# seongsujeong/MIMC3

Hardware: AMD Instinct MI355X
Metric: grid-points/s (DLC NCC match) (higher is better)
Workload: dtype u8

## Files before the change

### mimc3_amd/csrc/match_px_kernel.hip

```cpp
#include <hip/hip_runtime.h>
#include <type_traits>
#include <atomic>
#include <mutex>
#include <stdint.h>
#include <stdlib.h>
#include <stdio.h>
#include "match_kernel.h"
#include "sat_kernel.h"

#ifndef MIMC3_XY_ACC
#define MIMC3_XY_ACC 2
#endif
#ifndef MIMC3_SAT_DEFER
#define MIMC3_SAT_DEFER -1
#endif
#ifndef MIMC3_WN
#define MIMC3_WN 1
#endif
#ifndef MIMC3_NULL_FLAGS
#define MIMC3_NULL_FLAGS 1
#endif
#ifndef MIMC3_OPQ_SMALL
#define MIMC3_OPQ_SMALL 1
#endif
#ifndef MIMC3_FAST_REPLAY
#define MIMC3_FAST_REPLAY 1
#endif
#ifndef MIMC3_WIDE_REPLAY
#define MIMC3_WIDE_REPLAY 1
#endif
#ifndef MIMC3_GC
#define MIMC3_GC 1
#endif
#ifndef MIMC3_STAGE_KB
#define MIMC3_STAGE_KB 8
#endif
#ifndef MIMC3_EVEN_PITCH
#define MIMC3_EVEN_PITCH 0
#endif
#ifndef MIMC3_FAST_BATCH
#define MIMC3_FAST_BATCH 64
#endif

namespace mimc3 {

static constexpr float kUnknown = 3.0f;
static constexpr float kWanted = 4.0f;

__device__ __forceinline__ uint32_t dot4(uint32_t a, uint32_t b, uint32_t c) { return __builtin_amdgcn_udot4(a, b, c, false); }
__device__ __forceinline__ uint32_t alignb(uint32_t hi, uint32_t lo, uint32_t s) { return __builtin_amdgcn_alignbyte(hi, lo, s); }
__device__ __forceinline__ uint32_t nz80(uint32_t v) { return (((v & 0x7f7f7f7fu) + 0x7f7f7f7fu) | v) & 0x80808080u; }
typedef unsigned short nzff_us2_t __attribute__((ext_vector_type(2)));
__device__ __forceinline__ uint32_t nzff(uint32_t v)
{
    const uint32_t e = (v & 0x00ff00ffu) + 0x7fff7fffu;
    const nzff_us2_t k = {0x7f00, 0x7f00};
    const uint32_t o = __builtin_bit_cast(uint32_t, __builtin_elementwise_add_sat(__builtin_bit_cast(nzff_us2_t, v), k));
    return __builtin_amdgcn_perm(o, e, 0x0b090a08u);
}

template <int LPC>
__device__ __forceinline__ uint32_t group_sum(uint32_t v)
{
    int x = (int)v;
    x += __builtin_amdgcn_update_dpp(0, x, 0xB1, 0xF, 0xF, true);
    x += __builtin_amdgcn_update_dpp(0, x, 0x4E, 0xF, 0xF, true);
    if (LPC >= 8) x += __builtin_amdgcn_update_dpp(0, x, 0x141, 0xF, 0xF, true);
    if (LPC >= 16) x += __builtin_amdgcn_update_dpp(0, x, 0x140, 0xF, 0xF, true);
    if (LPC >= 32) x += __shfl_xor(x, 16, 64);
    if (LPC >= 64) x += __shfl_xor(x, 32, 64);
    return (uint32_t)x;
}
__device__ __forceinline__ int wave_sum_i(int v)
{
#pragma unroll
    for (int o = 32; o > 0; o >>= 1) v += __shfl_xor(v, o, 64);
    return v;
}

__device__ __forceinline__ void argmax_row16(float &v, int &i)
{
#define MIMC3_ARGMAX_STEP(ctrl)                                                                           \
    {                                                                                                     \
        const float ov = __int_as_float(__builtin_amdgcn_update_dpp(0, __float_as_int(v), ctrl, 0xF, 0xF, true)); \
        const int oi = __builtin_amdgcn_update_dpp(0, i, ctrl, 0xF, 0xF, true);                           \
        const bool t = (ov > v) || (ov == v && oi < i);                                                   \
        v = t ? ov : v; i = t ? oi : i;                                                                   \
    }
    MIMC3_ARGMAX_STEP(0xB1) MIMC3_ARGMAX_STEP(0x4E) MIMC3_ARGMAX_STEP(0x141) MIMC3_ARGMAX_STEP(0x140)
#undef MIMC3_ARGMAX_STEP
}

enum { M_FAST = 0, M_CHIPNULL = 1, M_GENERAL = 2, M_XY = 3, M_WN = 4, M_GC = 5 };

template <class S> struct AccT { uint32_t n; S sx, sy, sxx, syy, sxy; };

__device__ __forceinline__ double dpp_add_f64(double x, int ctrl_sel)
{
    const long long b = __double_as_longlong(x);
    int lo = (int)(b & 0xffffffffll), hi = (int)(b >> 32);
    int olo, ohi;
    switch (ctrl_sel) {
    case 0: olo = __builtin_amdgcn_update_dpp(0, lo, 0xB1, 0xF, 0xF, true); ohi = __builtin_amdgcn_update_dpp(0, hi, 0xB1, 0xF, 0xF, true); break;
    case 1: olo = __builtin_amdgcn_update_dpp(0, lo, 0x4E, 0xF, 0xF, true); ohi = __builtin_amdgcn_update_dpp(0, hi, 0x4E, 0xF, 0xF, true); break;
    case 2: olo = __builtin_amdgcn_update_dpp(0, lo, 0x141, 0xF, 0xF, true); ohi = __builtin_amdgcn_update_dpp(0, hi, 0x141, 0xF, 0xF, true); break;
    default: olo = __builtin_amdgcn_update_dpp(0, lo, 0x140, 0xF, 0xF, true); ohi = __builtin_amdgcn_update_dpp(0, hi, 0x140, 0xF, 0xF, true); break;
    }
    return x + __longlong_as_double(((long long)ohi << 32) | (unsigned int)olo);
}

struct PxU8 {
    static constexpr int BPP = 1, G = 4, LOG2G = 2;
    static constexpr bool SRC16 = false;
    static constexpr bool INTEGER = true;
    static constexpr bool SAT = true;
    static constexpr bool SATZ = false;
    static constexpr bool SAT_CHIP = true;
    static constexpr bool WN = true;
    typedef unsigned long long SatT;
    __device__ static __forceinline__ unsigned long long sat_s(SatT q) { return (uint32_t)q & ((1u << kSatSqShift8) - 1u); }
    __device__ static __forceinline__ unsigned long long sat_ss(SatT q) { return (uint32_t)(q >> kSatSqShift8) & ((1u << (kSatNullShift8 - kSatSqShift8)) - 1u); }
    __device__ static __forceinline__ int sat_nulls(SatT q) { return (int)(q >> kSatNullShift8); }
    __device__ static __forceinline__ void sat_win_sums(uint32_t &sy, uint32_t &syy, SatT q, int, int, int, double) { sy = (uint32_t)sat_s(q); syy = (uint32_t)sat_ss(q); }
    __device__ static __forceinline__ uint32_t px_at(const unsigned char *p) { return *p; }
    typedef uint32_t Sum;
    static constexpr uint32_t lowmask_c(int npx) { return npx >= 4 ? 0xffffffffu : ((1u << (8 * npx)) - 1u); }
    __device__ static __forceinline__ uint32_t lowmask(int npx) { return npx >= 4 ? 0xffffffffu : ((1u << (8 * npx)) - 1u); }
    __device__ static __forceinline__ int npx(uint32_t m) { return __popc(m & 0x01010101u); }
    __device__ static __forceinline__ int nbad(uint32_t v, uint32_t keep, float) { return npx(keep) - __popc(nz80(v) >> 7); }
    __device__ static __forceinline__ int nexcl(uint32_t v, uint32_t keep, float thr) { return nbad(v, keep, thr); }
    __device__ static __forceinline__ uint32_t sanitize(uint32_t a, float) { return a; }
    __device__ static __forceinline__ bool maybe_excl(uint32_t v, uint32_t keep, float) { return ((v - 0x01010101u) & ~v & 0x80808080u & keep) != 0u; }
    __device__ static __forceinline__ void chip_acc(Sum &sx, Sum &sxx, uint32_t a) { sx = dot4(a, 0x01010101u, sx); sxx = dot4(a, a, sxx); }
    template <int MODE, bool OPQ>
    __device__ static __forceinline__ void task(AccT<Sum> &acc, uint32_t a, uint32_t pad01, uint32_t padff, bool static_pad, uint32_t bw, float)
    {
        if (MODE == M_XY) {
            if (static_pad) acc.sxy = dot4(a, bw, acc.sxy); else acc.sy = dot4(a, bw, acc.sy);
            return;
        }
        if (MODE == M_WN) {
            const uint32_t am = a & nzff(bw);
            acc.sx = dot4(am, 0x01010101u, acc.sx);
            acc.sxx = dot4(am, a, acc.sxx);
            acc.sxy = dot4(a, bw, acc.sxy);
            return;
        }
        if (MODE == M_GC && static_pad) {
            const uint32_t mbff = nzff(bw);
            const uint32_t am = a & mbff;
            acc.n += (uint32_t)__popc(padff == 0xffffffffu ? mbff : (mbff & padff));
            acc.sx = dot4(am, 0x01010101u, acc.sx);
            acc.sy = dot4(pad01, bw, acc.sy);
            acc.sxy = dot4(a, bw, acc.sxy);
            acc.sxx = dot4(am, a, acc.sxx);
            acc.syy = dot4(padff == 0xffffffffu ? bw : (bw & padff), bw, acc.syy);
            return;
        }
        if (OPQ && !(MODE == M_FAST && static_pad)) asm volatile("" : "+v"(a));
        const uint32_t mf = (MODE == M_FAST && static_pad) ? padff : nzff(a);
        if (MODE == M_FAST) {
            const uint32_t m01 = static_pad ? pad01 : (mf & 0x01010101u);
            const uint32_t mff = static_pad ? padff : mf;
            acc.sy = dot4(m01, bw, acc.sy);
            acc.syy = dot4((static_pad && padff == 0xffffffffu) ? bw : (bw & mff), bw, acc.syy);
            acc.sxy = dot4(a, bw, acc.sxy);
        } else if (MODE == M_CHIPNULL) {
            const uint32_t bm = bw & mf;
            acc.sy = dot4(bm, 0x01010101u, acc.sy);
            acc.syy = dot4(bm, bw, acc.syy);
            acc.sxy = dot4(a, bw, acc.sxy);
        } else {
            const uint32_t mbff = nzff(bw);
            const uint32_t am = a & mbff, bm = bw & mf;
            acc.n += (uint32_t)__popc(mbff & mf);
            acc.sx = dot4(am, 0x01010101u, acc.sx);
            acc.sy = dot4(bm, 0x01010101u, acc.sy);
            acc.sxy = dot4(a, bw, acc.sxy);
            acc.sxx = dot4(am, a, acc.sxx);
            acc.syy = dot4(bm, bw, acc.syy);
        }
    }
    __device__ static __forceinline__ uint32_t n_units(uint32_t n) { return n >> 3; }
    template <int LPC> __device__ static __forceinline__ Sum gsum(Sum v) { return group_sum<LPC>(v); }
    typedef uint32_t Store;
    __device__ static __forceinline__ Store bits(Sum v) { return v; }
    __device__ static __forceinline__ float ncc(const Store *sp, double, double, int, int)
    {
        const double dn = (double)sp[0], dsx = (double)sp[1], dsy = (double)sp[2];
        const double num = dn * (double)sp[5] - dsx * dsy;
        const double den = sqrt((dn * (double)sp[3] - dsx * dsx) * (dn * (double)sp[4] - dsy * dsy));
        return (float)(num / den);
    }
};

typedef unsigned short us2_t __attribute__((ext_vector_type(2)));
__device__ __forceinline__ uint32_t dot2(uint32_t a, uint32_t b, uint32_t c)
{
    return __builtin_amdgcn_udot2(__builtin_bit_cast(us2_t, a), __builtin_bit_cast(us2_t, b), c, false);
}
__device__ __forceinline__ uint32_t nz8000(uint32_t v) { return (((v & 0x7fff7fffu) + 0x7fff7fffu) | v) & 0x80008000u; }
__device__ __forceinline__ uint32_t ffff_from8000(uint32_t t) { return t | (t - (t >> 15)); }
__device__ __forceinline__ unsigned long long dpp_add_u64(unsigned long long x, int ctrl_sel)
{
    int lo = (int)(uint32_t)x, hi = (int)(uint32_t)(x >> 32);
    int olo, ohi;
    switch (ctrl_sel) {
    case 0: olo = __builtin_amdgcn_update_dpp(0, lo, 0xB1, 0xF, 0xF, true); ohi = __builtin_amdgcn_update_dpp(0, hi, 0xB1, 0xF, 0xF, true); break;
    case 1: olo = __builtin_amdgcn_update_dpp(0, lo, 0x4E, 0xF, 0xF, true); ohi = __builtin_amdgcn_update_dpp(0, hi, 0x4E, 0xF, 0xF, true); break;
    case 2: olo = __builtin_amdgcn_update_dpp(0, lo, 0x141, 0xF, 0xF, true); ohi = __builtin_amdgcn_update_dpp(0, hi, 0x141, 0xF, 0xF, true); break;
    default: olo = __builtin_amdgcn_update_dpp(0, lo, 0x140, 0xF, 0xF, true); ohi = __builtin_amdgcn_update_dpp(0, hi, 0x140, 0xF, 0xF, true); break;
    }
    return x + (((unsigned long long)(uint32_t)ohi << 32) | (uint32_t)olo);
}
struct PxU16 {
    static constexpr int BPP = 2, G = 2, LOG2G = 1;
    static constexpr bool SRC16 = false;
    static constexpr bool INTEGER = true;
    static constexpr bool SAT = true;
    static constexpr bool SATZ = true;
    static constexpr bool SAT_CHIP = true;
    static constexpr bool WN = true;
    typedef unsigned long long SatT;
    __device__ static __forceinline__ unsigned long long sat_s(SatT q) { return q & ((1ull << kSatSqShift16) - 1ull); }
    __device__ static __forceinline__ unsigned long long sat_ss(SatT q) { return q >> kSatSqShift16; }
    __device__ static __forceinline__ int sat_nulls(SatT) { return 0; }
    __device__ static __forceinline__ void sat_win_sums(unsigned long long &sy, unsigned long long &syy, SatT q, int, int, int, double) { sy = sat_s(q); syy = sat_ss(q); }
    __device__ static __forceinline__ uint32_t px_at(const unsigned char *p) { return *reinterpret_cast<const unsigned short *>(p); }
    typedef unsigned long long Sum;
    static constexpr uint32_t lowmask_c(int npx) { return npx >= 2 ? 0xffffffffu : (npx == 1 ? 0x0000ffffu : 0u); }
    __device__ static __forceinline__ uint32_t lowmask(int npx) { return npx >= 2 ? 0xffffffffu : (npx == 1 ? 0x0000ffffu : 0u); }
    __device__ static __forceinline__ int npx(uint32_t m) { return __popc(m & 0x00010001u); }
    __device__ static __forceinline__ int nbad(uint32_t v, uint32_t keep, float) { return npx(keep) - __popc(nz8000(v) >> 15); }
    __device__ static __forceinline__ int nexcl(uint32_t v, uint32_t keep, float thr) { return nbad(v, keep, thr); }
    __device__ static __forceinline__ uint32_t sanitize(uint32_t a, float) { return a; }
// ... 186 lines not shown
        const double sxx = __longlong_as_double((long long)sp[3]), syy = __longlong_as_double((long long)sp[4]);
        const double sxy = __longlong_as_double((long long)sp[5]);
        const double num = dn * sxy - sx * sy;
        const double den = sqrt((dn * sxx - sx * sx) * (dn * syy - sy * sy));
        return (float)(num / den);
    }
};

struct PxF32i : PxF32 {
    static constexpr bool SAT = true, SATZ = false, SAT_CHIP = true;
    static constexpr bool WN = true;
    typedef Sat2 SatT;
    __device__ static __forceinline__ double sat_s(const SatT &q) { return (double)(q.a & ((1ull << kSatNullShiftF) - 1ull)); }
    __device__ static __forceinline__ double sat_ss(const SatT &q) { return (double)q.b; }
    __device__ static __forceinline__ int sat_nulls(const SatT &q) { return (int)(q.a >> kSatNullShiftF); }
    __device__ static __forceinline__ void sat_win_sums(double &sy, double &syy, const SatT &q, int, int, int, double sc) { sy = sat_s(q) * sc; syy = sat_ss(q) * (sc * sc); }
    template <int MODE, bool OPQ>
    __device__ static __forceinline__ void task(AccT<Sum> &acc, uint32_t au, uint32_t p01, uint32_t pff, bool static_pad, uint32_t bu, float thr)
    {
        if (MODE == M_XY) {
            const double pr = (double)(__uint_as_float(au) * __uint_as_float(bu));
            if (static_pad) acc.sxy += pr; else acc.sy += pr;
            return;
        }
        if (MODE == M_WN) {
            const float a = __uint_as_float(au), b = __uint_as_float(bu);
            const float a2 = (b != 0.0f) ? a : 0.0f;
            acc.sx += (double)a2; acc.sxx += (double)(a2 * a2); acc.sxy += (double)(a * b);
            return;
        }
        PxF32::template task<MODE, OPQ>(acc, au, p01, pff, static_pad, bu, thr);
    }
};

template <class P_, int OCW_, int LPC_, int NW_ = 1, int MINW_ = 2, bool CHL_ = false, bool MANY_ = false, bool COMPACT_ = false>
struct PxCfg {
    typedef P_ P;
    static constexpr bool COMPACT = COMPACT_;
    static constexpr bool SAT_DEFER = std::is_same<P_, PxU8>::value && NW_ == 1;
    static constexpr int MINW = MINW_;
    static constexpr int OCW = OCW_, LPC = LPC_;
    static constexpr int NW = NW_, NT = 64 * NW_;
    static constexpr int CW = 2 * OCW + 1, NPX = CW * CW;
    static constexpr int GPR = (CW + P::G - 1) / P::G;
    static constexpr bool SHORT = CW < LPC;
    static constexpr int RF = SHORT ? 1 : CW / LPC;
    static constexpr int REM = SHORT ? 0 : CW - RF * LPC;
    static constexpr int TT = (REM * GPR + LPC - 1) / LPC;
    static constexpr int LASTN = CW - P::G * (GPR - 1);
    static constexpr uint32_t LASTFF = P::lowmask_c(LASTN);
    static constexpr uint32_t LAST01 = LASTFF & 0x01010101u;
    static constexpr int CPR = 64 / LPC;
    static constexpr bool WN = P_::WN && (!std::is_same<P_, PxU8>::value || ((SHORT ? 1 : CW / LPC_) >= 2 && !((LPC_ >= 64) && P_::INTEGER)));
    static constexpr bool kOpqSmall = MIMC3_OPQ_SMALL && ((std::is_same<P_, PxU8>::value && OCW_ == 16) || (std::is_same<P_, PxU8o>::value && (OCW_ == 15 || OCW_ == 16)));
    static constexpr bool OPQ = LPC_ >= 64 || kOpqSmall;
    static constexpr bool SPARSE = (LPC_ >= 64) && P::INTEGER;
    static constexpr int CPITCH = 4 * GPR;
    static constexpr bool CHIP_LDS = CHL_;
    static constexpr bool CHIP_COPY = SPARSE || CHIP_LDS;
    static constexpr bool MANYP = MANY_;
    static constexpr bool REC = false;
    static constexpr bool SHORTCUT = !MANY_ && ((OCW_ == 16 && !std::is_same<P_, PxF32>::value) ||
                                                (OCW_ == 7 && (std::is_same<P_, PxU8>::value || std::is_same<P_, PxU8o>::value || std::is_same<P_, PxF32>::value)));
    static constexpr bool one_pad_task_per_lane()
    {
        for (int ln = 0; ln < LPC_; ln++) {
            int cnt = 0;
            for (int k = 0; k < TT; k++) {
                const int tt = ln + LPC_ * k;
                if (tt < REM * GPR && tt % GPR == GPR - 1) cnt++;
            }
            if (cnt > 1) return false;
        }
        return true;
    }
    static constexpr bool FULLTAIL = SPARSE && !CHIP_LDS && TT >= 4 && LASTN < P::G && one_pad_task_per_lane();
};
template <class C0>
struct PxRec : C0 {
    static constexpr bool REC = true;
};
static constexpr int kLwCap = 1024;
static constexpr int kLcCap = 512;

struct U8Point {
    int dx2, dy2, Dx2, Dy2, csx, csy, ncell;
    int sh;
    int PW;
    int zrow;
    float thr;
};

template <class C, int MODE, bool REDUCE = true, bool FULLTAIL = false>
__device__ __forceinline__ AccT<typename C::P::Sum> eval_round(const unsigned char *W, const U8Point &pt, int cx, int cy, int l,
                                          const uint32_t (&A)[C::RF > 0 ? C::RF : 1][C::GPR],
                                          const uint32_t (&AT)[C::TT > 0 ? C::TT : 1],
                                          const int (&toff)[C::TT > 0 ? C::TT : 1],
                                          AccT<typename C::P::Sum> acc = AccT<typename C::P::Sum>{0, 0, 0, 0, 0, 0},
                                          const unsigned char *CH = nullptr)
{
    typedef typename C::P P;
    [[maybe_unused]] const typename P::Sum sy_in = acc.sy;
    const int X = pt.sh + cx;
    const uint32_t s = (uint32_t)((X & (P::G - 1)) * P::BPP);
    const unsigned char *base = W + cy * pt.PW + 4 * (X >> P::LOG2G);
    constexpr int NLD = C::GPR + (P::G > 1 ? 1 : 0);
    if constexpr (C::CHIP_LDS) {
        constexpr int KC = 8;
#pragma unroll
        for (int i = 0; i < C::RF; i++) {
            const bool idle = C::SHORT && l >= C::CW;
            const uint32_t *rp = reinterpret_cast<const uint32_t *>(idle ? W + pt.zrow * pt.PW : base + (l + C::LPC * i) * pt.PW);
            const uint32_t *cp = reinterpret_cast<const uint32_t *>(CH + (idle ? 0 : (l + C::LPC * i)) * C::CPITCH);
#pragma unroll 1
            for (int j0 = 0; j0 < C::GPR - 1; j0 += KC) {
                uint32_t w[KC + 1], a[KC];
#pragma unroll
                for (int k = 0; k <= KC; k++) w[k] = rp[j0 + k];
#pragma unroll
                for (int k = 0; k < KC; k++) a[k] = (j0 + k < C::GPR - 1 && !idle) ? cp[j0 + k] : 0u;
#pragma unroll
                for (int k = 0; k < KC; k++) {
                    const uint32_t bw = (P::G > 1) ? alignb(w[k + 1], w[k], s) : w[k];
                    if (j0 + k < C::GPR - 1) P::template task<MODE, C::OPQ>(acc, a[k], 0x01010101u, 0xffffffffu, true, bw, pt.thr);
                }
            }
            {
                constexpr int j = C::GPR - 1;
                const uint32_t w0 = rp[j], w1 = (P::G > 1) ? rp[j + 1] : 0u;
                const uint32_t bw = (P::G > 1) ? alignb(w1, w0, s) : w0;
                const uint32_t av = idle ? 0u : cp[j];
                P::template task<MODE, C::OPQ>(acc, av, C::LAST01, C::LASTFF, true, bw, pt.thr);
            }
        }
    } else {
#pragma unroll
    for (int i = 0; i < C::RF; i++) {
        const uint32_t *rp = reinterpret_cast<const uint32_t *>(base + (l + C::LPC * i) * pt.PW);
        if (C::SHORT && l >= C::CW) rp = reinterpret_cast<const uint32_t *>(W + pt.zrow * pt.PW);
        uint32_t w[NLD];
#pragma unroll
        for (int j = 0; j < NLD; j++) w[j] = rp[j];
#pragma unroll
        for (int j = 0; j < C::GPR; j++) {
            const uint32_t bw = (P::G > 1) ? alignb(w[j + (P::G > 1 ? 1 : 0)], w[j], s) : w[j];
            const uint32_t p01 = (j == C::GPR - 1) ? C::LAST01 : 0x01010101u;
            const uint32_t pff = (j == C::GPR - 1) ? C::LASTFF : 0xffffffffu;
            if constexpr (MODE == M_XY) P::template task<M_XY, C::OPQ>(acc, A[i][j], 0, 0, (MIMC3_XY_ACC < 2) || ((i * C::GPR + j) & 1) == 0, bw, pt.thr);
            else P::template task<MODE, C::OPQ>(acc, A[i][j], p01, pff, true, bw, pt.thr);
        }
    }
    }
#pragma unroll
    for (int k = 0; k < C::TT; k++) {
        const uint32_t *rp = reinterpret_cast<const uint32_t *>(base + toff[k]);
        const uint32_t bw = (P::G > 1) ? alignb(rp[P::G > 1 ? 1 : 0], rp[0], s) : rp[0];
        uint32_t av = AT[k];
        if constexpr (C::CHIP_LDS) {
            const int tt = l + C::LPC * k;
            av = tt < C::REM * C::GPR ? *reinterpret_cast<const volatile uint32_t *>(CH + (C::RF * C::LPC + tt / C::GPR) * C::CPITCH + 4 * (tt % C::GPR)) : 0u;
        }
        if constexpr (MODE == M_XY) {
            P::template task<M_XY, C::OPQ>(acc, av, 0, 0, (MIMC3_XY_ACC < 2) || (k & 1) == 0, bw, pt.thr);
        }
        else if constexpr (FULLTAIL && MODE == M_FAST) {
            uint32_t bwt = bw;
            if (k == C::TT - 1 && (C::REM * C::GPR) % C::LPC != 0) bwt = (l + C::LPC * k < C::REM * C::GPR) ? bw : 0u;
            P::template task<M_FAST, C::OPQ>(acc, av, P::BPP == 1 ? 0x01010101u : 0x00010001u, 0xffffffffu, true, bwt, pt.thr);
        }
        else P::template task<MODE, C::OPQ>(acc, av, 0, 0, false, bw, pt.thr);
    }
    if constexpr (MODE == M_XY && MIMC3_XY_ACC >= 2) { acc.sxy += acc.sy - sy_in; acc.sy = sy_in; }
    if (MODE == M_GENERAL || MODE == M_GC) acc.n = P::n_units(acc.n);
    if (!REDUCE) return acc;
    acc.sxy = P::template gsum<C::LPC>(acc.sxy);
    if (MODE != M_XY && MODE != M_WN) { acc.sy = P::template gsum<C::LPC>(acc.sy); acc.syy = P::template gsum<C::LPC>(acc.syy); }
    if (MODE == M_WN) { acc.sx = P::template gsum<C::LPC>(acc.sx); acc.sxx = P::template gsum<C::LPC>(acc.sxx); }
    if (MODE == M_GENERAL || MODE == M_GC) {
        acc.n = group_sum<C::LPC>(acc.n); acc.sx = P::template gsum<C::LPC>(acc.sx); acc.sxx = P::template gsum<C::LPC>(acc.sxx);
    }
    return acc;
}

static constexpr int kStatW = 20;
#ifndef MIMC3_SUM_BATCH
#define MIMC3_SUM_BATCH 32
#endif
static constexpr int kSumBatch = MIMC3_SUM_BATCH;

#define MIMC3_STAMP(i)                                                                         \
    if (p.stats) {                                                                             \
        const unsigned long long t_now = __builtin_amdgcn_s_memtime();                         \
        if (threadIdx.x == 0) p.stats[kStatW * (size_t)blockIdx.x + i] += t_now - t_prev;                   \
        t_prev = t_now;                                                                        \
    }

template <class C>
__global__ __launch_bounds__(C::NT, C::MINW) void match_ncc_dlc_px(MatchU8Args p)
{
    typedef typename C::P P;
    typedef typename P::Sum Sum;
    constexpr bool kSat = P::SAT && !C::MANYP, kSatChip = P::SAT_CHIP && kSat, kSatZ = P::SATZ && kSat;
    unsigned long long t_prev = p.stats ? __builtin_amdgcn_s_memtime() : 0ull;
    extern __shared__ __attribute__((aligned(16))) unsigned char smem[];
    const int tid = threadIdx.x, lane = tid & 63, wave = tid >> 6;
    const int l = lane & (C::LPC - 1), grp = lane / C::LPC;
    constexpr int OCW = C::OCW, CW = C::CW, GPR = C::GPR, NT = C::NT, NW = C::NW;

    int gidx = blockIdx.x;
    constexpr bool kRec = C::REC;
    static_assert(!kRec || (std::is_same<P, PxU8>::value && !C::MANYP), "point records: the 8-bit policy's plain forms");
    [[maybe_unused]] uint32_t recw = 0u;
    auto rec = [&](int k) __attribute__((always_inline)) -> uint32_t { return (uint32_t)__builtin_amdgcn_readlane((int)recw, k); };
    if (kRec || p.point_list) {
        const int cnt = *p.point_count;
        if (gidx >= cnt) return;
        const int per = cnt >> 3;
        if (gidx < per * 8) gidx = (gidx & 7) * per + (gidx >> 3);
        if constexpr (kRec) {
            static_assert(sizeof(U8PointRec) == 64 && offsetof(U8PointRec, chipQ) == 40, "the dword numbers below");
            recw = reinterpret_cast<const uint32_t *>(p.point_recs + gidx)[lane & 15];
            if (rec(8) & kRecDone) return;
            gidx = (int)rec(0);
        } else gidx = p.point_list[gidx];
    } else {
        const int nb = gridDim.x, per = nb >> 3;
        if (per > 0 && gidx < per * 8) gidx = (gidx & 7) * per + (gidx >> 3);
    }
    if (gidx >= p.N) return;
    if (p.point_flags && p.point_flags[gidx] != (uint8_t)p.flag_value) return;
// ... 416 lines not shown
                    exc_chip += nzc;
                    if constexpr (C::SPARSE) {
                        if (wave == 0 && rowok && nzc) {
                            int at = atomicAdd(&qcnt[17], nzc);
                            if (at + nzc > kLcCap) qcnt[18] = 1;
                            else {
#pragma unroll
                                for (int k = 0; k < P::G; k++) {
                                    const uint32_t pm = P::lowmask(1) << (8 * P::BPP * k);
                                    if ((pff & pm) && !(a & pm)) nl_put(Lc, at++, (uint32_t)(P::G * j + k), (uint32_t)(l + C::LPC * i));
                                }
                            }
                        }
                    }
                }
            }
#pragma unroll
            for (int k = 0; k < C::TT; k++) {
                const int tt = l + C::LPC * k;
                const bool on = tt < C::REM * GPR;
                const int j = on ? tt % GPR : 0;
                const uint32_t pff = on ? ((j == GPR - 1) ? C::LASTFF : 0xffffffffu) : 0u;
                if (P::maybe_excl(AT[k], pff, pt.thr)) {
                    bad_chip += P::nbad(AT[k], pff, pt.thr);
                    const int nzc = P::nexcl(AT[k], pff, pt.thr);
                    exc_chip += nzc;
                    if constexpr (C::FULLTAIL || (kSat && C::SPARSE)) {
                        if (wave == 0 && on && nzc) {
                            int at = atomicAdd(&qcnt[17], nzc);
                            if (at + nzc > kLcCap) qcnt[18] = 1;
                            else {
#pragma unroll
                                for (int q = 0; q < P::G; q++) {
                                    const uint32_t pm = P::lowmask(1) << (8 * P::BPP * q);
                                    if ((pff & pm) && !(AT[k] & pm)) nl_put(Lc, at++, (uint32_t)(P::G * j + q), (uint32_t)(C::RF * C::LPC + tt / GPR));
                                }
                            }
                        }
                    }
                }
            }
        }
        if constexpr (kSatChip) {
            bad_chip = exc_chip = chip_nulls;
            SX = (Sum)P::sat_s(chipQ); SXX = (Sum)P::sat_ss(chipQ);
            if constexpr (!P::INTEGER) { SX = (Sum)((double)SX * sc_chip); SXX = (Sum)((double)SXX * (sc_chip * sc_chip)); }
        } else {
            bad_chip = (int)group_sum<C::LPC>((uint32_t)bad_chip); exc_chip = (int)group_sum<C::LPC>((uint32_t)exc_chip);
            SX = P::template gsum<C::LPC>(SX); SXX = P::template gsum<C::LPC>(SXX);
        }
    }
    const uint32_t NV = (uint32_t)(C::NPX - exc_chip);
    const int clean_mode = (exc_chip == 0) ? M_FAST : M_CHIPNULL;
    MIMC3_STAMP(1)
    if (p.debug_stop == 2) { if (tid == 0) p.out[3 * (size_t)gidx] = (float)((uint32_t)P::bits(SX) + (uint32_t)P::bits(SXX) + bad_chip + A[0][0] + AT[0]); return; }
    __syncthreads();
    const bool sparse_on = C::SPARSE && qcnt[18] == 0;
    const int nLw = sparse_on ? qcnt[16] : 0, nLc = sparse_on ? qcnt[17] : 0;
    (void)nLw; (void)nLc;
    if (p.stats && tid == 0) {
        p.stats[kStatW * (size_t)blockIdx.x + 11] += sparse_on ? 1 : 0;
        p.stats[kStatW * (size_t)blockIdx.x + 12] += (unsigned)nLw; p.stats[kStatW * (size_t)blockIdx.x + 13] += (unsigned)nLc;
    }

    {
        const float max_ratio = 0.8f;
        const float rc = (float)bad_chip / (float)(CW * CW);
        const float rw = (float)bad_win / (float)(pt.Dx2 * pt.Dy2);
        if (rc > max_ratio || rw > max_ratio) {
            if (tid == 0) {
                const float nanv = __builtin_nanf("");
                p.out[3 * (size_t)gidx + 0] = nanv;
                p.out[3 * (size_t)gidx + 1] = nanv;
                p.out[3 * (size_t)gidx + 2] = -3.0f;
            }
            return;
        }
    }
    static_assert(OCW >= 2, "T4 cmap cells are reachable by the fit only when ocw == 1; not instantiated");
    auto box_clean = [&](int cx, int cy) __attribute__((always_inline)) -> bool {
        if (!full_win && (cx == pt.csx - 2 || cy == pt.csy - 2)) return false;
        if (win_clean) return true;
        return (cx > nbx1) || (cx + CW - 1 < nbx0) || (cy > nby1) || (cy + CW - 1 < nby0);
    };

    auto request = [&](int cx, int cy) __attribute__((always_inline)) {
        if (!claim(cx, cy)) return;
        if constexpr (C::COMPACT) {
            const int slot = atomicAdd(&qcnt[2], 1);
            if (slot >= p.lds_nslot) { qcnt[3] = 1; return; }
            give_slot(cx, cy, slot);
        }
        const bool cl = box_clean(cx, cy);
        const uint32_t q = (uint32_t)atomicAdd(&qcnt[0], cl ? 1 : (1 << 16));
        const int ia = (int)(q & 0xffffu), ib = (int)(q >> 16);
        if (ia + ib + 1 > lcap) { qcnt[3] = 1; return; }
        const uint16_t packed = (uint16_t)((cy << 8) | cx);
        if (cl) list[ia] = packed; else list[lcap - 1 - ib] = packed;
    };
    auto inside = [&](int pu, int pvv) __attribute__((always_inline)) -> bool {
        return !(pu - OCW <= 1 || pu + OCW >= pt.Dx2 - 1 || pvv - OCW <= 1 || pvv + OCW >= pt.Dy2 - 1);
    };
    auto scan9 = [&](int cu, int cv, float &sm) __attribute__((always_inline)) -> int {
        float v[9];
#pragma unroll
        for (int j = 0; j < 9; j++) v[j] = lookup(cu + (j / 3 - 1) - OCW, cv + (j % 3 - 1) - OCW);
// ... 20 lines not shown
        if constexpr (C::COMPACT) {
            slot0 = atomicAdd(&qcnt[2], __popc(won));
            if (slot0 + __popc(won) > p.lds_nslot) { qcnt[3] = 1; return; }
        }
        const uint32_t row_t4 = (!full_win && cy0 == pt.csy - 3) ? 4u : 0u;
        const bool col_t4 = !full_win && cx0 == pt.csx - 3;
        uint32_t cl;
        if (win_clean) {
            cl = (7u & ~row_t4) * (col_t4 ? 0x09u : 0x49u);
        } else {
            uint32_t row_ok = 0u;
#pragma unroll
            for (int k = 0; k < 3; k++) {
                const int cy = cy0 + k - 1;
                row_ok |= (cy > nby1 || cy + CW - 1 < nby0) ? (1u << k) : 0u;
            }
            cl = 0u;
#pragma unroll
            for (int i = 0; i < 3; i++) {
                const int cx = cx0 + i - 1;
                const bool col_ok = cx > nbx1 || cx + CW - 1 < nbx0;
                const uint32_t part = (i == 2 && col_t4) ? 0u : ((col_ok ? 7u : row_ok) & ~row_t4);
                cl |= part << (3 * i);
            }
        }
        const uint32_t wa = won & cl, wb = won & ~cl;
        const int na = __popc(wa), nb = __popc(wb);
        const uint32_t q = (uint32_t)atomicAdd(&qcnt[0], na | (nb << 16));
        int ia = (int)(q & 0xffffu), ib = (int)(q >> 16);
        if (ia + ib + na + nb > lcap) { qcnt[3] = 1; return; }
#pragma unroll
        for (int j = 0; j < 9; j++) {
            if (!((won >> j) & 1u)) continue;
            const int cx = cx0 + (j / 3 - 1), cy = cy0 + (j % 3 - 1);
            const uint16_t packed = (uint16_t)((cy << 8) | cx);
            if ((wa >> j) & 1u) list[ia++] = packed; else list[lcap - 1 - ib++] = packed;
            if constexpr (C::COMPACT) give_slot(cx, cy, slot0++);
        }
    };
    for (int k = tid; k < npiv; k += NT) {
        const int pu = pivs[2 * k] + pt.dx2, pvv = pivs[2 * k + 1] + pt.dy2;
        if (!inside(pu, pvv)) continue;
        request9(pu - OCW, pvv - OCW);
    }
    __syncthreads();
    if (p.debug_stop == 3) return;
    MIMC3_STAMP(2)

    constexpr bool kAPark = (C::LPC >= 32) && P::INTEGER;
    constexpr bool kSatDefer = MIMC3_SAT_DEFER < 0 ? C::SAT_DEFER : (MIMC3_SAT_DEFER != 0);
    auto evaluate = [&](const uint16_t *ids, int dir, int cnt, int mode) __attribute__((always_inline)) {
        const bool dirty_list = (mode == M_GENERAL);
        const bool wn_ok = kSat && C::WN && MIMC3_WN && dirty_list && exc_chip == 0;
        uint32_t ew[4] = {0xffffffffu, 0xffffffffu, 0xffffffffu, 0xffffffffu}, ec[2] = {0xffffffffu, 0xffffffffu};
        if constexpr (C::SPARSE) {
            if (sparse_on && cnt > 0) {
                if (dirty_list) {
#pragma unroll
                    for (int k = 0; k < 4; k++) if (l + k * C::LPC < nLw) ew[k] = nl_get(Lw, l + k * C::LPC);
                }
#pragma unroll
                for (int k = 0; k < 2; k++) if (l + k * C::LPC < nLc) ec[k] = nl_get(Lc, l + k * C::LPC);
            }
        }
        constexpr int kFastBatch = (6 * kSumBatch < MIMC3_FAST_BATCH) ? 6 * kSumBatch : MIMC3_FAST_BATCH;
        const bool one_word = kSat && !kAPark && NT == 64 && mode == M_FAST && kFastBatch > kSumBatch;
        const int batch_cells = one_word ? kFastBatch : kSumBatch;
        for (int b0 = 0; b0 < cnt; b0 += batch_cells) {
            const int nb = (cnt - b0) < batch_cells ? (cnt - b0) : batch_cells;
            [[maybe_unused]] SatT cellQ{}, q00{}, q01{}, q10{}, q11{};
            [[maybe_unused]] int cellZ = 0;
            if constexpr (kSat) {
                const bool need = mode == M_FAST || (C::SPARSE && sparse_on) || (dirty_list && wn_ok);
                if (need && tid < nb) {
                    const uint32_t pk = ids[dir * (b0 + tid)];
                    const SatT *r0 = sat_win + (size_t)(wv0 + (int)((pk >> 8) & 0xffu)) * p.sat_ws + (wu0 + (int)(pk & 0xffu)), *r1 = r0 + (size_t)CW * p.sat_ws;
                    q00 = r0[0]; q01 = r0[CW]; q10 = r1[0]; q11 = r1[CW];
                    if (!kSatDefer) cellQ = q11 - q01 - q10 + q00;
                    if constexpr (kSatZ) {
                        if (dirty_list) cellZ = (int)sat_box(satz_win, p.sat_ws, wu0 + (int)(pk & 0xffu), wv0 + (int)((pk >> 8) & 0xffu), CW, CW);
                    }
                }
            }
            [[maybe_unused]] unsigned char *nzf = reinterpret_cast<unsigned char *>(&qcnt[24]);
            constexpr bool kNullFlags = C::SPARSE && kSat && !kSatDefer && kSumBatch <= 32 && MIMC3_NULL_FLAGS;
            const bool flags_on = kNullFlags && 3 * CW * CW <= pt.Dx2 * pt.Dy2;
            if constexpr (kNullFlags) {
                if (dirty_list && sparse_on && flags_on) {
                    if (tid < nb) nzf[tid] = (unsigned char)((kSatZ ? cellZ : P::sat_nulls(cellQ)) != 0);
                    __syncthreads();
                }
            }
            for (int r0 = 0; r0 < nb; r0 += C::CPR * NW) {
                const int slot = r0 + wave * C::CPR + grp;
                const bool on = slot < nb;
                const uint32_t pk = on ? ids[dir * (b0 + slot)] : 0x00000101u;
                const int cx = (int)(pk & 0xffu), cy = (int)((pk >> 8) & 0xffu);
                AccT<Sum> acc;
                bool six = dirty_list;
                bool done = false;
                bool wn_round = false;
                if constexpr (C::SPARSE) {
                    if (sparse_on && !(dirty_list && !full_win && (cx == pt.csx - 2 || cy == pt.csy - 2))) {
                        AccT<Sum> a0{0, 0, 0, 0, 0, 0};
                        uint32_t cn = 0;
                        Sum csx = 0, csxx = 0, csy = 0, csyy = 0;
                        auto corr_w = [&](const uint32_t (&e)[4]) __attribute__((always_inline)) {
                            uint32_t av[4];
                            bool in[4];
#pragma unroll
                            for (int k = 0; k < 4; k++) {
                                const int ddx = (int)(e[k] & 0xffffu) - cx, ddy = (int)(e[k] >> 16) - cy;
                                in[k] = (unsigned)ddx < (unsigned)CW && (unsigned)ddy < (unsigned)CW;
                                av[k] = P::px_at(CH + (in[k] ? (int)__umul24(ddy, C::CPITCH) + ddx * P::BPP : 0));
                            }
#pragma unroll
                            for (int k = 0; k < 4; k++) {
                                const uint32_t a1 = in[k] ? av[k] : 0u;
                                cn += a1 ? 1u : 0u; csx += a1; csxx += (Sum)__umul24(a1, a1);
                            }
                        };
                        const unsigned char *Wc = W + cy * pt.PW + (pt.sh + cx) * P::BPP;
                        auto corr_c = [&](const uint32_t (&e)[2]) __attribute__((always_inline)) {
                            uint32_t bv[2];
#pragma unroll
                            for (int k = 0; k < 2; k++) {
                                const bool ok = e[k] != 0xffffffffu;
                                bv[k] = P::px_at(Wc + (ok ? (int)__umul24(e[k] >> 16, pt.PW) + (int)(e[k] & 0xffffu) * P::BPP : 0));
                                bv[k] = ok ? bv[k] : 0u;
                            }
#pragma unroll
                            for (int k = 0; k < 2; k++) { csy += bv[k]; csyy += (Sum)__umul24(bv[k], bv[k]); }
                        };
                        bool wnull = dirty_list;
                        if constexpr (kNullFlags) { if (flags_on) wnull = dirty_list && on && nzf[slot] != 0; }
                        six = wnull;
                        if (wnull) {
                            corr_w(ew);
                            for (int i0 = l + 4 * C::LPC; i0 < nLw; i0 += 4 * C::LPC) {
                                uint32_t e[4];
#pragma unroll
                                for (int k = 0; k < 4; k++) e[k] = (i0 + k * C::LPC < nLw) ? nl_get(Lw, i0 + k * C::LPC) : 0xffffffffu;
                                corr_w(e);
                            }
                        }
                        if (nLc > 0) {
                            corr_c(ec);
                            for (int i0 = l + 2 * C::LPC; i0 < nLc; i0 += 2 * C::LPC) {
                                uint32_t e[2];
#pragma unroll
                                for (int k = 0; k < 2; k++) e[k] = (i0 + k * C::LPC < nLc) ? nl_get(Lc, i0 + k * C::LPC) : 0xffffffffu;
                                corr_c(e);
                            }
                        }
                        if constexpr (C::FULLTAIL && !kSat) {
                            const int X = pt.sh + cx;
                            const uint32_t sft = (uint32_t)((X & (P::G - 1)) * P::BPP);
                            const uint32_t *rp = reinterpret_cast<const uint32_t *>(W + cy * pt.PW + 4 * (X >> P::LOG2G) + (padoff >= 0 ? padoff : 0));
                            const uint32_t pb = padoff >= 0 ? (alignb(rp[1], rp[0], sft) & ~C::LASTFF) : 0u;
                            P::chip_acc(csy, csyy, pb);
                        }
                        constexpr bool kFold = sizeof(Sum) == 4;
                        if (kFold) { a0.sy = (Sum)0 - csy; a0.syy = (Sum)0 - csyy; }
                        acc = eval_round<C, kSat ? M_XY : M_FAST, false, C::FULLTAIL>(W, pt, cx, cy, l, A, AT, toff, a0, CH);
                        if (!kFold) { acc.sy -= csy; acc.syy -= csyy; }
                        acc.n = 0u - cn; acc.sx = (Sum)0 - csx; acc.sxx = (Sum)0 - csxx;
                        done = true;
                    } else {
                        six = dirty_list;
                    }
                }
                if (!done) {
                    if (mode == M_FAST) acc = eval_round<C, kSat ? M_XY : M_FAST, !kAPark>(W, pt, cx, cy, l, A, AT, toff, AccT<Sum>{0, 0, 0, 0, 0, 0}, CH);
                    else if (mode == M_CHIPNULL) acc = eval_round<C, M_CHIPNULL, !kAPark>(W, pt, cx, cy, l, A, AT, toff, AccT<Sum>{0, 0, 0, 0, 0, 0}, CH);
                    else {
                        if constexpr (kSat) {
                            const bool t4 = on && !full_win && (cx == pt.csx - 2 || cy == pt.csy - 2);
                            wn_round = wn_ok && __ballot(t4) == 0ull;
                        }
                        if (kSat && wn_round) acc = eval_round<C, kSat ? M_WN : M_GENERAL, !kAPark>(W, pt, cx, cy, l, A, AT, toff, AccT<Sum>{0, 0, 0, 0, 0, 0}, CH);
                        else if (MIMC3_GC && exc_chip == 0) acc = eval_round<C, M_GC, !kAPark>(W, pt, cx, cy, l, A, AT, toff, AccT<Sum>{0, 0, 0, 0, 0, 0}, CH);
                        else acc = eval_round<C, M_GENERAL, !kAPark>(W, pt, cx, cy, l, A, AT, toff, AccT<Sum>{0, 0, 0, 0, 0, 0}, CH);
                    }
                }
                Store *sp = sums + 6 * slot;
                if constexpr (kAPark) {
                    const bool lead = on && (l & 15) == 0;
                    const Sum rsxy = P::template gsum<16>(acc.sxy);
                    if (lead) atomicAdd(&sp[5], P::bits(rsxy));
                    if (!kSat || (done ? nLc > 0 : (mode != M_FAST && !wn_round))) {
                        const Sum rsy = P::template gsum<16>(acc.sy), rsyy = P::template gsum<16>(acc.syy);
                        if (lead) { atomicAdd(&sp[2], P::bits(rsy)); atomicAdd(&sp[4], P::bits(rsyy)); }
                    }
                    if (six) {
                        const Sum rsx = P::template gsum<16>(acc.sx), rsxx = P::template gsum<16>(acc.sxx);
                        if (lead) { atomicAdd(&sp[1], P::bits(rsx)); atomicAdd(&sp[3], P::bits(rsxx)); }
                        if (!wn_round) {
                            const uint32_t rn = group_sum<16>(acc.n);
                            if (lead) atomicAdd(&sp[0], (Store)rn);
                        }
                    }
                } else {
                    if (kSat && mode == M_FAST) {
                        if (on && l == 0) { if (one_word) sums[slot] = P::bits(acc.sxy); else sp[5] = P::bits(acc.sxy); }
                    } else {
                        if (mode != M_GENERAL) { acc.n = NV; acc.sx = SX; acc.sxx = SXX; }
                        if (on && l == 0) {
                            if (kSat && wn_round) { sp[1] = P::bits(acc.sx); sp[3] = P::bits(acc.sxx); sp[5] = P::bits(acc.sxy); }
                            else { sp[0] = (Store)acc.n; sp[1] = P::bits(acc.sx); sp[2] = P::bits(acc.sy); sp[3] = P::bits(acc.sxx); sp[4] = P::bits(acc.syy); sp[5] = P::bits(acc.sxy); }
                        }
                    }
                }
            }
            __syncthreads();
            if (tid < nb) {
                if (kSatDefer) cellQ = q11 - q01 - q10 + q00;
                const uint32_t pk = ids[dir * (b0 + tid)];
                const int cx = (int)(pk & 0xffu), cy = (int)((pk >> 8) & 0xffu);
                Store *sp = sums + 6 * tid;
                Store v[6] = {0, 0, 0, 0, 0, 0};
                if (one_word) v[5] = sums[tid];
                else { v[0] = sp[0]; v[1] = sp[1]; v[2] = sp[2]; v[3] = sp[3]; v[4] = sp[4]; v[5] = sp[5]; }
                bool wn_cell = false;
                if constexpr (kSat) {
                    if (wn_ok) {
                        const bool t4 = !full_win && (cx == pt.csx - 2 || cy == pt.csy - 2);
                        const unsigned long long tm = __ballot(t4);
                        wn_cell = ((tm >> (tid & ~(C::CPR - 1))) & ((1ull << C::CPR) - 1ull)) == 0ull;
                        if (C::SPARSE && sparse_on) wn_cell = false;
                    }
                    if (wn_cell) {
                        Sum ty = 0, tyy = 0;
                        const int z = kSatZ ? cellZ : P::sat_nulls(cellQ);
                        if (p.stats && z == 0) atomicAdd(&p.stats[kStatW * (size_t)blockIdx.x + 15], 1ull);
                        P::sat_win_sums(ty, tyy, cellQ, z, kb, C::NPX, sc_win);
                        v[0] = (Store)(uint32_t)(C::NPX - z); v[2] = P::bits(ty); v[4] = P::bits(tyy);
                    }
                }
                if constexpr (kAPark) {
                    const bool dense = dirty_list && !(C::SPARSE && sparse_on && !(!full_win && (cx == pt.csx - 2 || cy == pt.csy - 2)));
                    (void)wn_cell;
                    if (!dense) { v[0] += (Store)NV; v[1] += P::bits(SX); v[3] += P::bits(SXX); }
                    if constexpr (kSat) {
                        const bool sparse_cell = C::SPARSE && sparse_on && !(dirty_list && !full_win && (cx == pt.csx - 2 || cy == pt.csy - 2));
                        if (sparse_cell || mode == M_FAST) {
                            Sum ty = 0, tyy = 0;
                            P::sat_win_sums(ty, tyy, cellQ, cellZ, kb, C::NPX, sc_win);
                            v[2] += P::bits(ty); v[4] += P::bits(tyy);
                        }
                    }
                    if (C::SPARSE) v[0] = (Store)(uint32_t)v[0];
#pragma unroll
                    for (int k = 0; k < 6; k++) sp[k] = 0;
                }
                if constexpr (kSat && !kAPark) {
                    if (mode == M_FAST) {
                        Sum ty = 0, tyy = 0;
                        P::sat_win_sums(ty, tyy, cellQ, 0, kb, C::NPX, sc_win);
                        v[0] = (Store)NV; v[1] = P::bits(SX); v[2] = P::bits(ty); v[3] = P::bits(SXX); v[4] = P::bits(tyy);
                    }
                }
                store_ncc(cx, cy, P::ncc(v, sc_chip, sc_win, ka, kb));
            }
            __syncthreads();
        }
    };
    constexpr int kSpecRounds = 16;
    const int kLookahead = p.lookahead;
    int stage = 0;
    int su = 0, sv = 0;
    bool alive = false;
    float smax = -2.0f;
    if (wave == 0 && lane < npiv) {
        su = pivs[2 * lane] + pt.dx2; sv = pivs[2 * lane + 1] + pt.dy2;
        alive = inside(su, sv);
    }
    const int start_u = su, start_v = sv;
    unsigned long long traj = 0ull;
    int nsc = 0;
    bool replay_generic = false;
    bool cut = false;
    uint32_t xdone = 0u;
    bool xpending = false;
    unsigned long long *trajL = reinterpret_cast<unsigned long long *>(smem + (C::MANYP ? p.lds_off_traj : 0));
    unsigned char *tinfo = reinterpret_cast<unsigned char *>(trajL + npiv);
    unsigned char *Tl = tinfo + npiv;
    (void)xdone; (void)xpending; (void)trajL; (void)tinfo; (void)Tl;
    int k = 0, pu = 0, pvv = 0, du = 0, dv = 0, newncc = 0;
    bool fresh = true;
    float nccmax = -2.0f, best = -2.0f;
    int peak_u = pt.dx2, peak_v = pt.dy2;

    for (int guard = 0; guard <= pt.ncell + 16; guard++) {
        if (qcnt[3]) {
            if (tid == 0) p.ovf_list[atomicAdd(p.ovf_count, 1)] = gidx;
            return;
        }
        {
            const int nA = qcnt[0] & 0xffff, nB = (int)((uint32_t)qcnt[0] >> 16);
            if (p.stats && tid == 0) {
                p.stats[kStatW * (size_t)blockIdx.x + 8] += nA; p.stats[kStatW * (size_t)blockIdx.x + 9] += nB;
                p.stats[kStatW * (size_t)blockIdx.x + 10] += (nA + nB) ? 1 : 0;
            }
            __syncthreads();
            if (tid == 0) qcnt[0] = 0;
            evaluate(list, 1, nA, clean_mode);
            evaluate(list + lcap - 1, -1, nB, M_GENERAL);
            __syncthreads();
        }
        if (p.debug_stop == 4) return;
        MIMC3_STAMP(3)
        auto step = [&]() __attribute__((always_inline)) -> int {
// ... 806 lines not shown
```

Measured before the change: 100.0 million.

## Use SAT window sums with sparse chip-null corrections in u8 match rounds

```diff
diff --git a/mimc3_amd/csrc/match_px_kernel.hip b/mimc3_amd/csrc/match_px_kernel.hip
--- a/mimc3_amd/csrc/match_px_kernel.hip
+++ b/mimc3_amd/csrc/match_px_kernel.hip
@@ -16,6 +16,9 @@
 #endif
 #ifndef MIMC3_WN
 #define MIMC3_WN 1
+#endif
+#ifndef MIMC3_CN_SKIP
+#define MIMC3_CN_SKIP 1
 #endif
 #ifndef MIMC3_NULL_FLAGS
 #define MIMC3_NULL_FLAGS 1
@@ -91,7 +94,7 @@
 #undef MIMC3_ARGMAX_STEP
 }
 
-enum { M_FAST = 0, M_CHIPNULL = 1, M_GENERAL = 2, M_XY = 3, M_WN = 4, M_GC = 5 };
+enum { M_FAST = 0, M_CHIPNULL = 1, M_GENERAL = 2, M_XY = 3, M_WN = 4, M_GC = 5, M_XYC = 6, M_WNC = 7 };
 
 template <class S> struct AccT { uint32_t n; S sx, sy, sxx, syy, sxy; };
 
@@ -181,6 +184,16 @@
             acc.syy = dot4(bm, bw, acc.syy);
         }
     }
+    template <bool WIN, bool OPQ>
+    __device__ static __forceinline__ void cn_task(Sum &csy, Sum &csyy, uint32_t &cj, uint32_t a, uint32_t pff, uint32_t bw)
+    {
+        if (OPQ) asm volatile("" : "+v"(a));
+        const uint32_t za = ~nzff(a) & pff;
+        const uint32_t bz = bw & za;
+        csy = dot4(bz, 0x01010101u, csy);
+        csyy = dot4(bz, bw, csyy);
+        if (WIN) cj += (uint32_t)__popc(za & ~nzff(bw));
+    }
     __device__ static __forceinline__ uint32_t n_units(uint32_t n) { return n >> 3; }
     template <int LPC> __device__ static __forceinline__ Sum gsum(Sum v) { return group_sum<LPC>(v); }
     typedef uint32_t Store;
@@ -473,6 +486,8 @@
     static constexpr uint32_t LAST01 = LASTFF & 0x01010101u;
     static constexpr int CPR = 64 / LPC;
     static constexpr bool WN = P_::WN && (!std::is_same<P_, PxU8>::value || ((SHORT ? 1 : CW / LPC_) >= 2 && !((LPC_ >= 64) && P_::INTEGER)));
+    static constexpr bool CN_ELIGIBLE = MIMC3_CN_SKIP && std::is_same<P_, PxU8>::value && NW_ == 1 && OCW_ == 16 && LPC_ == 16 && !CHL_ && !MANY_;
+    static constexpr bool CN_SKIP = false;
     static constexpr bool kOpqSmall = MIMC3_OPQ_SMALL && ((std::is_same<P_, PxU8>::value && OCW_ == 16) || (std::is_same<P_, PxU8o>::value && (OCW_ == 15 || OCW_ == 16)));
     static constexpr bool OPQ = LPC_ >= 64 || kOpqSmall;
     static constexpr bool SPARSE = (LPC_ >= 64) && P::INTEGER;
@@ -500,6 +515,7 @@
 template <class C0>
 struct PxRec : C0 {
     static constexpr bool REC = true;
+    static constexpr bool CN_SKIP = C0::CN_ELIGIBLE;
 };
 static constexpr int kLwCap = 1024;
 static constexpr int kLcCap = 512;
@@ -518,9 +534,13 @@
                                           const uint32_t (&AT)[C::TT > 0 ? C::TT : 1],
                                           const int (&toff)[C::TT > 0 ? C::TT : 1],
                                           AccT<typename C::P::Sum> acc = AccT<typename C::P::Sum>{0, 0, 0, 0, 0, 0},
-                                          const unsigned char *CH = nullptr)
+                                          const unsigned char *CH = nullptr, uint32_t cmask = 0u)
 {
     typedef typename C::P P;
+    constexpr bool kCnMode = MODE == M_XYC || MODE == M_WNC;
+    static_assert(!kCnMode || (!C::CHIP_LDS && !C::SHORT && C::RF * C::GPR + C::TT <= 32), "flag mask: one bit per task index");
+    [[maybe_unused]] typename P::Sum csy = 0, csyy = 0;
+    [[maybe_unused]] uint32_t cj = 0u;
     [[maybe_unused]] const typename P::Sum sy_in = acc.sy;
     const int X = pt.sh + cx;
     const uint32_t s = (uint32_t)((X & (P::G - 1)) * P::BPP);
@@ -567,8 +587,11 @@
             const uint32_t bw = (P::G > 1) ? alignb(w[j + (P::G > 1 ? 1 : 0)], w[j], s) : w[j];
             const uint32_t p01 = (j == C::GPR - 1) ? C::LAST01 : 0x01010101u;
             const uint32_t pff = (j == C::GPR - 1) ? C::LASTFF : 0xffffffffu;
-            if constexpr (MODE == M_XY) P::template task<M_XY, C::OPQ>(acc, A[i][j], 0, 0, (MIMC3_XY_ACC < 2) || ((i * C::GPR + j) & 1) == 0, bw, pt.thr);
-            else P::template task<MODE, C::OPQ>(acc, A[i][j], p01, pff, true, bw, pt.thr);
+            if constexpr (MODE == M_XY || MODE == M_XYC) P::template task<M_XY, C::OPQ>(acc, A[i][j], 0, 0, (MIMC3_XY_ACC < 2) || ((i * C::GPR + j) & 1) == 0, bw, pt.thr);
+            else P::template task<MODE == M_WNC ? M_WN : MODE, C::OPQ>(acc, A[i][j], p01, pff, true, bw, pt.thr);
+            if constexpr (kCnMode) {
+                if ((cmask >> (i * C::GPR + j)) & 1u) P::template cn_task<MODE == M_WNC, C::OPQ>(csy, csyy, cj, A[i][j], pff, bw);
+            }
         }
     }
     }
@@ -581,7 +604,7 @@
             const int tt = l + C::LPC * k;
             av = tt < C::REM * C::GPR ? *reinterpret_cast<const volatile uint32_t *>(CH + (C::RF * C::LPC + tt / C::GPR) * C::CPITCH + 4 * (tt % C::GPR)) : 0u;
         }
-        if constexpr (MODE == M_XY) {
+        if constexpr (MODE == M_XY || MODE == M_XYC) {
             P::template task<M_XY, C::OPQ>(acc, av, 0, 0, (MIMC3_XY_ACC < 2) || (k & 1) == 0, bw, pt.thr);
         }
         else if constexpr (FULLTAIL && MODE == M_FAST) {
@@ -589,14 +612,23 @@
             if (k == C::TT - 1 && (C::REM * C::GPR) % C::LPC != 0) bwt = (l + C::LPC * k < C::REM * C::GPR) ? bw : 0u;
             P::template task<M_FAST, C::OPQ>(acc, av, P::BPP == 1 ? 0x01010101u : 0x00010001u, 0xffffffffu, true, bwt, pt.thr);
         }
-        else P::template task<MODE, C::OPQ>(acc, av, 0, 0, false, bw, pt.thr);
-    }
-    if constexpr (MODE == M_XY && MIMC3_XY_ACC >= 2) { acc.sxy += acc.sy - sy_in; acc.sy = sy_in; }
+        else P::template task<MODE == M_WNC ? M_WN : MODE, C::OPQ>(acc, av, 0, 0, false, bw, pt.thr);
+        if constexpr (kCnMode) {
+            if ((cmask >> (C::RF * C::GPR + k)) & 1u) {
+                const int tt = l + C::LPC * k;
+                const uint32_t tff = tt < C::REM * C::GPR ? ((tt % C::GPR == C::GPR - 1) ? C::LASTFF : 0xffffffffu) : 0u;
+                P::template cn_task<MODE == M_WNC, C::OPQ>(csy, csyy, cj, av, tff, bw);
+            }
+        }
+    }
+    if constexpr ((MODE == M_XY || MODE == M_XYC) && MIMC3_XY_ACC >= 2) { acc.sxy += acc.sy - sy_in; acc.sy = sy_in; }
     if (MODE == M_GENERAL || MODE == M_GC) acc.n = P::n_units(acc.n);
+    if constexpr (kCnMode) { acc.sy = csy; acc.syy = csyy; acc.n = P::n_units(cj); }
     if (!REDUCE) return acc;
     acc.sxy = P::template gsum<C::LPC>(acc.sxy);
     if (MODE != M_XY && MODE != M_WN) { acc.sy = P::template gsum<C::LPC>(acc.sy); acc.syy = P::template gsum<C::LPC>(acc.syy); }
-    if (MODE == M_WN) { acc.sx = P::template gsum<C::LPC>(acc.sx); acc.sxx = P::template gsum<C::LPC>(acc.sxx); }
+    if (MODE == M_WN || MODE == M_WNC) { acc.sx = P::template gsum<C::LPC>(acc.sx); acc.sxx = P::template gsum<C::LPC>(acc.sxx); }
+    if (MODE == M_WNC) acc.n = group_sum<C::LPC>(acc.n);
     if (MODE == M_GENERAL || MODE == M_GC) {
         acc.n = group_sum<C::LPC>(acc.n); acc.sx = P::template gsum<C::LPC>(acc.sx); acc.sxx = P::template gsum<C::LPC>(acc.sxx);
     }
@@ -1119,6 +1151,26 @@
     }
     const uint32_t NV = (uint32_t)(C::NPX - exc_chip);
     const int clean_mode = (exc_chip == 0) ? M_FAST : M_CHIPNULL;
+    constexpr bool kCn = kSat && C::CN_SKIP && !((C::LPC >= 32) && P::INTEGER);
+    [[maybe_unused]] uint32_t cn_mask = 0u;
+    if constexpr (kCn) {
+        if (exc_chip != 0) {
+#pragma unroll
+            for (int i = 0; i < C::RF; i++) {
+#pragma unroll
+                for (int j = 0; j < GPR; j++) {
+                    const bool z = P::maybe_excl(A[i][j], (j == GPR - 1) ? C::LASTFF : 0xffffffffu, pt.thr);
+                    cn_mask |= (__ballot(z) != 0ull) ? (1u << (i * GPR + j)) : 0u;
+                }
+            }
+#pragma unroll
+            for (int k = 0; k < C::TT; k++) {
+                const int tt = l + C::LPC * k;
+                const uint32_t tff = tt < C::REM * GPR ? ((tt % GPR == GPR - 1) ? C::LASTFF : 0xffffffffu) : 0u;
+                cn_mask |= (__ballot(P::maybe_excl(AT[k], tff, pt.thr)) != 0ull) ? (1u << (C::RF * GPR + k)) : 0u;
+            }
+        }
+    }
     MIMC3_STAMP(1)
     if (p.debug_stop == 2) { if (tid == 0) p.out[3 * (size_t)gidx] = (float)((uint32_t)P::bits(SX) + (uint32_t)P::bits(SXX) + bad_chip + A[0][0] + AT[0]); return; }
     __syncthreads();
@@ -1245,6 +1297,8 @@
     auto evaluate = [&](const uint16_t *ids, int dir, int cnt, int mode) __attribute__((always_inline)) {
         const bool dirty_list = (mode == M_GENERAL);
         const bool wn_ok = kSat && C::WN && MIMC3_WN && dirty_list && exc_chip == 0;
+        const bool cn_ok = kCn && dirty_list && exc_chip != 0;
+        const bool cn_clean = kCn && mode == M_CHIPNULL;
         uint32_t ew[4] = {0xffffffffu, 0xffffffffu, 0xffffffffu, 0xffffffffu}, ec[2] = {0xffffffffu, 0xffffffffu};
         if constexpr (C::SPARSE) {
             if (sparse_on && cnt > 0) {
@@ -1264,7 +1318,7 @@
             [[maybe_unused]] SatT cellQ{}, q00{}, q01{}, q10{}, q11{};
             [[maybe_unused]] int cellZ = 0;
             if constexpr (kSat) {
-                const bool need = mode == M_FAST || (C::SPARSE && sparse_on) || (dirty_list && wn_ok);
+                const bool need = mode == M_FAST || (C::SPARSE && sparse_on) || (dirty_list && wn_ok) || cn_ok || cn_clean;
                 if (need && tid < nb) {
                     const uint32_t pk = ids[dir * (b0 + tid)];
                     const SatT *r0 = sat_win + (size_t)(wv0 + (int)((pk >> 8) & 0xffu)) * p.sat_ws + (wu0 + (int)(pk & 0xffu)), *r1 = r0 + (size_t)CW * p.sat_ws;
@@ -1365,13 +1419,19 @@
                 }
                 if (!done) {
                     if (mode == M_FAST) acc = eval_round<C, kSat ? M_XY : M_FAST, !kAPark>(W, pt, cx, cy, l, A, AT, toff, AccT<Sum>{0, 0, 0, 0, 0, 0}, CH);
-                    else if (mode == M_CHIPNULL) acc = eval_round<C, M_CHIPNULL, !kAPark>(W, pt, cx, cy, l, A, AT, toff, AccT<Sum>{0, 0, 0, 0, 0, 0}, CH);
+                    else if (mode == M_CHIPNULL) {
+                        if constexpr (kCn) acc = eval_round<C, M_XYC, !kAPark>(W, pt, cx, cy, l, A, AT, toff, AccT<Sum>{0, 0, 0, 0, 0, 0}, CH, cn_mask);
+                        else acc = eval_round<C, M_CHIPNULL, !kAPark>(W, pt, cx, cy, l, A, AT, toff, AccT<Sum>{0, 0, 0, 0, 0, 0}, CH);
+                    }
                     else {
                         if constexpr (kSat) {
                             const bool t4 = on && !full_win && (cx == pt.csx - 2 || cy == pt.csy - 2);
-                            wn_round = wn_ok && __ballot(t4) == 0ull;
+                            wn_round = (wn_ok || cn_ok) && __ballot(t4) == 0ull;
                         }
-                        if (kSat && wn_round) acc = eval_round<C, kSat ? M_WN : M_GENERAL, !kAPark>(W, pt, cx, cy, l, A, AT, toff, AccT<Sum>{0, 0, 0, 0, 0, 0}, CH);
+                        if (kCn && wn_round && cn_ok) {
+                            if constexpr (kCn) acc = eval_round<C, M_WNC, !kAPark>(W, pt, cx, cy, l, A, AT, toff, AccT<Sum>{0, 0, 0, 0, 0, 0}, CH, cn_mask);
+                        }
+                        else if (kSat && wn_round) acc = eval_round<C, kSat ? M_WN : M_GENERAL, !kAPark>(W, pt, cx, cy, l, A, AT, toff, AccT<Sum>{0, 0, 0, 0, 0, 0}, CH);
                         else if (MIMC3_GC && exc_chip == 0) acc = eval_round<C, M_GC, !kAPark>(W, pt, cx, cy, l, A, AT, toff, AccT<Sum>{0, 0, 0, 0, 0, 0}, CH);
                         else acc = eval_round<C, M_GENERAL, !kAPark>(W, pt, cx, cy, l, A, AT, toff, AccT<Sum>{0, 0, 0, 0, 0, 0}, CH);
                     }
@@ -1399,7 +1459,8 @@
                     } else {
                         if (mode != M_GENERAL) { acc.n = NV; acc.sx = SX; acc.sxx = SXX; }
                         if (on && l == 0) {
-                            if (kSat && wn_round) { sp[1] = P::bits(acc.sx); sp[3] = P::bits(acc.sxx); sp[5] = P::bits(acc.sxy); }
+                            if (cn_clean) { sp[2] = P::bits(acc.sy); sp[4] = P::bits(acc.syy); sp[5] = P::bits(acc.sxy); }
+                            else if (kSat && wn_round && !cn_ok) { sp[1] = P::bits(acc.sx); sp[3] = P::bits(acc.sxx); sp[5] = P::bits(acc.sxy); }
                             else { sp[0] = (Store)acc.n; sp[1] = P::bits(acc.sx); sp[2] = P::bits(acc.sy); sp[3] = P::bits(acc.sxx); sp[4] = P::bits(acc.syy); sp[5] = P::bits(acc.sxy); }
                         }
                     }
@@ -1416,7 +1477,7 @@
                 else { v[0] = sp[0]; v[1] = sp[1]; v[2] = sp[2]; v[3] = sp[3]; v[4] = sp[4]; v[5] = sp[5]; }
                 bool wn_cell = false;
                 if constexpr (kSat) {
-                    if (wn_ok) {
+                    if (wn_ok || cn_ok) {
                         const bool t4 = !full_win && (cx == pt.csx - 2 || cy == pt.csy - 2);
                         const unsigned long long tm = __ballot(t4);
                         wn_cell = ((tm >> (tid & ~(C::CPR - 1))) & ((1ull << C::CPR) - 1ull)) == 0ull;
@@ -1427,7 +1488,14 @@
                         const int z = kSatZ ? cellZ : P::sat_nulls(cellQ);
                         if (p.stats && z == 0) atomicAdd(&p.stats[kStatW * (size_t)blockIdx.x + 15], 1ull);
                         P::sat_win_sums(ty, tyy, cellQ, z, kb, C::NPX, sc_win);
-                        v[0] = (Store)(uint32_t)(C::NPX - z); v[2] = P::bits(ty); v[4] = P::bits(tyy);
+                        bool plain = true;
+                        if constexpr (kCn) {
+                            if (cn_ok) {
+                                v[0] = (Store)((uint32_t)(C::NPX - exc_chip - z) + (uint32_t)v[0]); v[2] = P::bits(ty) - v[2]; v[4] = P::bits(tyy) - v[4];
+                                plain = false;
+                            }
+                        }
+                        if (plain) { v[0] = (Store)(uint32_t)(C::NPX - z); v[2] = P::bits(ty); v[4] = P::bits(tyy); }
                     }
                 }
                 if constexpr (kAPark) {
@@ -1451,6 +1519,13 @@
                         Sum ty = 0, tyy = 0;
                         P::sat_win_sums(ty, tyy, cellQ, 0, kb, C::NPX, sc_win);
                         v[0] = (Store)NV; v[1] = P::bits(SX); v[2] = P::bits(ty); v[3] = P::bits(SXX); v[4] = P::bits(tyy);
+                    }
+                    if constexpr (kCn) {
+                        if (cn_clean) {
+                            Sum ty = 0, tyy = 0;
+                            P::sat_win_sums(ty, tyy, cellQ, 0, kb, C::NPX, sc_win);
+                            v[0] = (Store)NV; v[1] = P::bits(SX); v[2] = P::bits(ty) - v[2]; v[3] = P::bits(SXX); v[4] = P::bits(tyy) - v[4];
+                        }
                     }
                 }
                 store_ncc(cx, cy, P::ncc(v, sc_chip, sc_win, ka, kb));
```

After: 103.2 million, median of 6. 3.2% higher.
